# amirhajibabaei/AutoForce

Measured on AMD Instinct MI355X. Metric: MD-step atoms*steps/sec (SGPR predict: NL + descriptors + K_nm + E/F/stress + covloss); `value`: a Langevin MD loop on the device, every step from the forces of the one before (sgpr_md_run; --steps dependent steps between two fences); `value_resident_frames`: steps over independent frames resident i, higher is better.
Workload: dtype f64

## Files before the change

### autoforce_amd/csrc/api.hip

```cpp
#include <math.h>
#include <stdarg.h>
#include <stdio.h>
#include <stdlib.h>
#include <string.h>

#include <algorithm>
#include <numeric>

#include <dlfcn.h>
#include <unistd.h>
#include <rccl/rccl.h>

#include "../../include/sgpr_hip.h"
#include "sgpr_internal.h"
#include "nl_grid.inc"
#include <cmath>
#include <limits>

static thread_local char g_err[512] = "";
static int fail(int code, const char *fmt, ...)
{
    va_list ap;
    va_start(ap, fmt);
    vsnprintf(g_err, sizeof(g_err), fmt, ap);
// ... 1242 lines not shown
    if (const char *e = getenv("SGPR_ROWS16_MB")) h->rows16_mb = std::max(1, atoi(e));
    if (const char *e = getenv("SGPR_ROWS16_MIN")) h->rows16_min = std::max(1, atoi(e));
    {
        int ncu = 0;
        if (hipDeviceGetAttribute(&ncu, hipDeviceAttributeMultiprocessorCount, h->device) == hipSuccess && ncu >= 8) h->cus_per_xcd = ncu / 8;
    }
    if (getenv("SGPR_STAMPS")) { h->d_stamps.alloc(8 * 4096); h->d_stamps2.alloc(8 * 8192); }
    if (const char *e = getenv("SGPR_QR_KEEP")) h->qr_keep_mode = std::min(std::max(atoi(e), 0), 2);
    *out = h;
    return SGPR_OK;
}

static void drop_graph(sgpr_model *h)
{
    if (h->gexec) (void)hipGraphExecDestroy(h->gexec);
    h->gexec = nullptr;
}

extern "C" void sgpr_destroy(sgpr_model *h)
{
    if (!h) return;
    (void)hipSetDevice(h->device);
    (void)hipDeviceSynchronize();
    if (h->d_stamps.p && h->t_knm.n) {
        std::vector<long long> st(8 * h->t_knm.n);
        (void)hipMemcpy(st.data(), h->d_stamps.p, sizeof(long long) * st.size(), hipMemcpyDeviceToHost);
        double pro = 0, loop = 0, epi = 0; int n = 0; long long t0 = 1LL << 62, t1 = 0;
        for (size_t b = 0; b < h->t_knm.n; b++) {
            if (st[8 * b + 3] <= 0) continue;
            loop += st[8 * b + 1] - st[8 * b]; epi += st[8 * b + 2] - st[8 * b + 1]; n++;
            t0 = std::min(t0, st[8 * b]); t1 = std::max(t1, st[8 * b + 2]);
        }
        fprintf(stderr, "[sgpr stamps] K_nm gemm: %d tiles, start->loop end %.0f cyc, epilogue %.0f cyc, first start->last end %lld cyc\n",
                n, loop / std::max(n, 1), epi / std::max(n, 1), t1 - t0);
        (void)pro;
        if (const char *path = getenv("SGPR_STAMPS_FILE")) {
            if (FILE *f = fopen(path, "w")) {
                for (size_t b = 0; b < h->t_knm.n; b++)
                    fprintf(f, "knm %zu %lld %lld %lld %lld %lld %lld\n", b, st[8 * b], st[8 * b + 1], st[8 * b + 2], st[8 * b + 3], st[8 * b + 4], st[8 * b + 5]);
                std::vector<long long> s2(8 * std::min<size_t>(h->t_wcov.n, 8192));
                if (h->d_stamps2.p && !s2.empty()) {
                    (void)hipMemcpy(s2.data(), h->d_stamps2.p, sizeof(long long) * s2.size(), hipMemcpyDeviceToHost);
                    for (size_t b = 0; b < s2.size() / 8; b++)
                        fprintf(f, "wcov %zu %lld %lld %lld %lld %lld %lld\n", b, s2[8 * b], s2[8 * b + 1], s2[8 * b + 2], s2[8 * b + 3], s2[8 * b + 4], s2[8 * b + 5]);
                }
                fclose(f);
            }
        }
    }
    if (h->d_pstamps.p && h->N > 0) {
        const int N = h->N;
        std::vector<long long> st((size_t)16 * N);
        (void)hipMemcpy(st.data(), h->d_pstamps.p, sizeof(long long) * st.size(), hipMemcpyDeviceToHost);
        for (int pass = 0; pass < 2; pass++) {
            double d[7] = {0, 0, 0, 0, 0, 0, 0};
            long long t0 = 1LL << 62, t1 = 0;
            int cntw = 0;
            const int np = pass == 0 ? 6 : 3;
            for (int i = 0; i < h->cnt; i++) {
                const long long *w = st.data() + ((size_t)pass * N + i) * 8;
                if (w[0] <= 0 || w[np - 1] <= 0) continue;
                for (int k = 0; k + 1 < np; k++) d[k] += (double)(w[k + 1] - w[k]);
                t0 = std::min(t0, w[0]); t1 = std::max(t1, w[np - 1]);
                cntw++;
            }
            fprintf(stderr, "[sgpr stamps] %s: %d waves, cycles per phase:", pass == 0 ? "list+forward (sweep, sort, list out, tiles, c+spectrum)" : "reverse (dE/dc, pairs)", cntw);
            for (int k = 0; k + 1 < np; k++) fprintf(stderr, " %.0f", d[k] / std::max(cntw, 1));
            fprintf(stderr, "; first start -> last end %lld\n", t1 - t0);
            if (pass == 0) {
                double e[3] = {0, 0, 0};
                for (int i = 0; i < h->cnt; i++) {
                    const long long *w = st.data() + (size_t)i * 8;
                    if (w[0] <= 0 || w[5] <= 0) continue;
                    e[0] += (double)(w[3] - w[0]); e[1] += (double)(w[4] - w[3]); e[2] += (double)(w[5] - w[4]);
                }
                fprintf(stderr, "[sgpr stamps]    as a reuse step: list filter %.0f | c (radial, harmonics, MFMA) %.0f | spectrum + rows out %.0f\n",
                        e[0] / std::max(cntw, 1), e[1] / std::max(cntw, 1), e[2] / std::max(cntw, 1));
            }
        }
    }
    h->d_pstamps.release();
    drop_graph(h);
    for (auto e : h->ev) (void)hipEventDestroy(e);
    DevBuf<int> *ib[] = {&h->d_ind_slot, &h->d_ind_nn, &h->d_qoff, &h->d_perm, &h->d_slot, &h->d_aoff, &h->d_lslot,
                         &h->d_lnn, &h->d_bin_of, &h->d_bin_count, &h->d_nn_raw, &h->d_nn,
                         &h->d_nbr_j, &h->d_nbr_shift, &h->d_stat, &h->d_shear, &h->d_kslot, &h->d_aux,
                         &h->d_flag, &h->d_ncand, &h->d_cand_j, &h->d_cand_code, &h->d_cidx};
    for (auto b : ib) b->release();
    DevBuf<double> *db[] = {&h->d_radii, &h->d_Pm, &h->d_PmT, &h->d_pm_norm, &h->d_M, &h->d_mu, &h->d_choli,
                            &h->d_vs_sqrt, &h->d_gpart, &h->d_pos_in, &h->d_cell_in, &h->d_pos, &h->d_Pn, &h->d_norm, &h->d_C, &h->d_prec, &h->d_G,
                            &h->d_K, &h->d_Aw, &h->d_W, &h->d_F, &h->d_virpart, &h->d_Epart, &h->d_csq, &h->d_packed,
                            &h->d_rows_ones, &h->d_rows_out, &h->d_rows_ke, &h->d_L, &h->d_R1, &h->d_edit_tmp,
                            &h->d_rows_bG, &h->d_rows_bF, &h->d_rows_bV, &h->d_rows_kepart, &h->d_design, &h->d_qr_A, &h->d_qr_work};
    for (auto b : db) b->release();
    h->d_rows_cols.release();
    h->d_rows_rowof.release(); h->d_rows_qoff.release(); h->d_rows_vpart.release();
    if (h->pin) (void)hipHostFree(h->pin);
    if (h->pin_old) (void)hipHostFree(h->pin_old);
    if (h->md.halt_host) (void)hipHostFree(h->md.halt_host);
    if (h->md.mark) (void)hipHostFree(h->md.mark);
    if (h->md.scal_pin) (void)hipHostFree(h->md.scal_pin);
    {
        MdState &m = h->md;
        DevBuf<double> *mdb[] = {&m.X, &m.V, &m.P, &m.KE, &m.mass, &m.sig, &m.noise, &m.noise_raw, &m.cell, &m.scal_d};
        for (auto b : mdb) b->release();
        m.halt.release();
// ... 1615 lines not shown
```

### autoforce_amd/csrc/descriptor.hip

```cpp
#include "sgpr_internal.h"
#include "gemm_tile.inc"

__constant__ HarmCoef c_hc;

void upload_harm_coef(const HarmCoef &hc) { (void)hipMemcpyToSymbol(HIP_SYMBOL(c_hc), &hc, sizeof(HarmCoef)); }

#define SQRT2 1.4142135623730951
typedef double v4d __attribute__((ext_vector_type(4)));

__device__ __forceinline__ void wave_sync()
{
    __builtin_amdgcn_fence(__ATOMIC_RELEASE, "wavefront");
    __builtin_amdgcn_wave_barrier();
    __builtin_amdgcn_fence(__ATOMIC_ACQUIRE, "wavefront");
}

__device__ __forceinline__ double uniform(double v)
{
    const int lo = __builtin_amdgcn_readfirstlane(__double2loint(v));
    const int hi = __builtin_amdgcn_readfirstlane(__double2hiint(v));
    return __hiloint2double(hi, lo);
}

template <typename T>
__device__ __forceinline__ const T *launder(const T *p)
{
    asm volatile("" : "+s"(p));
    return p;
}

__device__ __forceinline__ double wave_sum(double v)
{
#pragma unroll
    for (int o = 32; o > 0; o >>= 1) v += __shfl_xor(v, o, 64);
    return v;
}

__device__ __forceinline__ int xcd_quad(int b, int n, int R)
{
    if (R <= 0) return b;
    const int grp = 8 * R, g0 = b / grp * grp;
    if (g0 + grp > n) return b;
    const int r = b - g0;
    return g0 + (r & 7) * R + (r >> 3);
}

template <int LMAX>
struct Harm {
    static constexpr int L1 = LMAX + 1, LL = L1 * L1;
    double A[L1], B[L1], q[L1][L1];
    double x, y, z, rho;
    const HarmCoef *hc = &c_hc;

    __device__ __forceinline__ void prepare(double x_, double y_, double z_)
    {
        x = x_; y = y_; z = z_;
        rho = x * x + y * y + z * z;
        A[0] = 1.0; B[0] = 0.0;
#pragma unroll
        for (int m = 1; m <= LMAX; m++) {
            A[m] = x * A[m - 1] - y * B[m - 1];
            B[m] = y * A[m - 1] + x * B[m - 1];
        }
        q[0][0] = hc->y00;
#pragma unroll
        for (int l = 1; l <= LMAX; l++) {
#pragma unroll
            for (int m = 0; m <= l - 2; m++)
                q[l][m] = hc->al[l][m] * (z * q[l - 1][m] + rho * hc->bl[l][m] * q[l - 2][m]);
            q[l][l - 1] = hc->cl[l] * z * q[l - 1][l - 1];
            q[l][l] = hc->dl[l] * q[l - 1][l - 1];
        }
    }

    __device__ __forceinline__ void eval(double x_, double y_, double z_, double *Y)
    {
        prepare(x_, y_, z_);
#pragma unroll
        for (int l = 0; l <= LMAX; l++) {
            Y[l * l] = q[l][0];
#pragma unroll
// ... 174 lines not shown

template <bool ENV>
__device__ __forceinline__ void load_neighbor(const DescArgs &a, int gi, int ia, int t, const double *pi,
                                              const double *cell, double r[3], int &s, int &j)
{
    if constexpr (ENV) {
        const int64_t e = a.env_ptr[ia] + t;
        r[0] = a.env_r[3 * e]; r[1] = a.env_r[3 * e + 1]; r[2] = a.env_r[3 * e + 2];
        s = a.env_slot[e];
        j = -1;
    } else {
        const size_t e = (size_t)gi * a.maxnn + t;
        j = a.nbr_j[e];
        const int code = a.nbr_shift[e];
        const double s0 = (double)(int)(int8_t)(code & 0xff);
        const double s1 = (double)(int)(int8_t)((code >> 8) & 0xff);
        const double s2 = (double)(int)(int8_t)((code >> 16) & 0xff);
#pragma unroll
        for (int k = 0; k < 3; k++)
            r[k] = a.pos[3 * (size_t)j + k] - pi[k] + (s0 * cell[k] + s1 * cell[3 + k] + s2 * cell[6 + k]);
        s = (code >> 24) & 0xff;
    }
}

template <int NMAX>
__device__ __forceinline__ void radial_ex(double d, double u, double rc, double irc, double ex, double *f, double &g,
                                          double &dg)
{
    const double ud = u * d;
    const double step = ud < rc ? 1.0 : 0.0;
    const double qq = 1.0 - ud * irc;
    const double cut = step * qq * qq;
    const double dcut = step * (-2.0 * qq * irc) * u;
    g = cut * ex;
    dg = dcut * ex - d * g;
    const double rho = d * d;
    double pw = g;
#pragma unroll
    for (int n = 0; n <= NMAX; n++) { f[n] = pw; pw *= rho; }
}

template <int NMAX>
__device__ __forceinline__ void radial(double d, double u, double rc, double *f, double &g, double &dg, double &ex)
{
    ex = exp(-0.5 * d * d);
    radial_ex<NMAX>(d, u, rc, 1.0 / rc, ex, f, g, dg);
}

template <int LMAX, int NMAX>
struct WaveLds {
    static constexpr int L1 = LMAX + 1, N1 = NMAX + 1, LL = L1 * L1, LLP = LL + 1, NSLOT = N1 * LL;
    static constexpr int CH = 48;
    static constexpr int TILE_D = CH * N1 + CH * LLP;
};

template <int LMAX, int NMAX, int ST, bool ENV>
__global__ __launch_bounds__(256) void desc_fwd_kernel(DescArgs a)
{
    using WL = WaveLds<LMAX, NMAX>;
    constexpr int N1 = WL::N1, LL = WL::LL, LLP = WL::LLP, NSLOT = WL::NSLOT;
    constexpr int SPL = (NSLOT + 63) / 64;
    extern __shared__ double smem[];
    const int wave = threadIdx.x >> 6, lane = threadIdx.x & 63;
    const int ia = blockIdx.x * 4 + wave;
    if (ia >= a.N) return;
    const int gi = a.first + ia * a.stride;
    constexpr int CH = WL::CH;
    const int perwave = WL::TILE_D + ST * NSLOT + 64 / 2;
    double *fl = smem + (size_t)wave * perwave;
    double *Yl = fl + CH * N1;
    double *cl = Yl + CH * LLP;
    int *sl = (int *)(cl + ST * NSLOT);

    int nn;
    double pi[3] = {0, 0, 0}, cell[9];
    if constexpr (ENV) {
        nn = (int)(a.env_ptr[ia + 1] - a.env_ptr[ia]);
    } else {
        nn = a.nn[gi];
#pragma unroll
        for (int k = 0; k < 3; k++) pi[k] = a.pos[3 * (size_t)gi + k];
#pragma unroll
        for (int k = 0; k < 9; k++) cell[k] = a.cell[k];
    }

    bool shear = false;
    if (nn > CH) {
        bool near = false;
        for (int t0 = 0; t0 < nn; t0 += 64) {
            const int t = t0 + lane;
            if (t < nn) {
                double r[3]; int s, j;
                load_neighbor<ENV>(a, gi, ia, t, pi, cell, r, s, j);
                const double u = unit_of<ST>(a, s);
                const double tol = SGPR_TINY_ANGLE * fabs(r[2] / u);
                near |= (fabs(r[0] / u) < tol) && (fabs(r[1] / u) < tol);
            }
        }
        shear = __any(near);
    }

    double acc[ST][SPL];
#pragma unroll
    for (int s = 0; s < ST; s++)
#pragma unroll
        for (int k = 0; k < SPL; k++) acc[s][k] = 0.0;
// ... 106 lines not shown
                nrm2 += pv[k][l] * pv[k][l];
            }
        }
    }
    nrm2 = wave_sum(nrm2);
    const double nrm = sqrt(nrm2);
    const double inv = nn > 0 ? 1.0 / (nrm + SGPR_EPS) : 0.0;
#pragma unroll
    for (int k = 0; k < MAXP; k++) {
        const int pr = lane + 64 * k;
        if (pr < npair) {
#pragma unroll
            for (int l = 0; l < L1; l++) a.Pn[(size_t)ia * a.Dpad + pr * L1 + l] = pv[k][l] * inv;
        }
    }
    for (int e = a.Dc + lane; e < a.Dpad; e += 64) a.Pn[(size_t)ia * a.Dpad + e] = 0.0;
    if (lane == 0) {
        a.norm[ia] = nn > 0 ? nrm : 0.0;
        if (a.shear) a.shear[ia] = shear ? 1 : 0;
    }
}

#define NL_SORT_MAX 256
#ifndef NL_STEPS
#define NL_STEPS 4
#endif

struct NlArgs {
    const NlGrid *grid;
    const int *bin_of, *kslot, *bin_count;
    int cap;
    const BinRec *b_rec;
    const BinAux *b_aux;
    int *nn, *nn_local, *nn_raw, *nbr_j, *nbr_shift, *aux;
    unsigned short *T;
    int t_stride;
    int *stat;
    const int *flag;
    double rc_list;
    int *ncand, *cand_j, *cand_code, *cidx;
    unsigned long long *hm;
    int hmw;
};

#ifdef SGPR_PHASE_STAMPS
#define PHASE_STAMP(K) if (a.stamps && lane == 0) a.stamps[(size_t)ia * 8 + (K)] = (long long)__builtin_amdgcn_s_memtime()
#else
#define PHASE_STAMP(K)
#endif

template <int LMAX, int NMAX, int ST>
struct FwdLds {
    using WL = WaveLds<LMAX, NMAX>;
    static constexpr int CH = WL::CH;
    static constexpr int BINL = NL_SORT_MAX + NL_SORT_MAX / 2, HIT0 = BINL + 2 * 64;
    static constexpr int NLV = HIT0 + 4 * CH;
    static constexpr int FWV = CH * WL::N1 + CH * WL::LLP + CH / 2;
    static constexpr int P4V = ST * WL::NSLOT;
    static constexpr int RA = (NLV > FWV ? (NLV > P4V ? NLV : P4V) : (FWV > P4V ? FWV : P4V));
    static constexpr int PW = 4 * CH + RA;
};

template <int LMAX, int NMAX, int ST>
__global__ __launch_bounds__(256, 4) void nl_fwd_kernel(DescArgs a, NlArgs n)
{
    using WL = WaveLds<LMAX, NMAX>;
    using FL = FwdLds<LMAX, NMAX, ST>;
    constexpr int N1 = WL::N1, LL = WL::LL, LLP = WL::LLP, NSLOT = WL::NSLOT, CH = WL::CH;
    constexpr int UC = ST * N1, CBS = (UC + 15) / 16, RBL = (LL + 15) / 16;
    extern __shared__ double smem[];
    const int wave = __builtin_amdgcn_readfirstlane(threadIdx.x >> 6), lane = threadIdx.x & 63;
    const int ia = xcd_quad((int)blockIdx.x, (int)gridDim.x, a.xq) * 4 + wave;
    if (ia >= a.N) return;
    const int i = a.first + ia * a.stride;
    double *wbase = smem + (size_t)wave * FL::PW;
    double *hit1 = wbase;
    double *RA = wbase + 4 * CH;
    unsigned long long *keys = (unsigned long long *)RA;
    int *hq = (int *)(RA + NL_SORT_MAX);
    int4 *binl = (int4 *)(RA + FL::BINL);
    double *hit0 = RA + FL::HIT0;
    double *fl = RA;
    double *Yl = fl + CH * N1;
    int *sl = (int *)(Yl + CH * LLP);
    double *cl = RA;

    PHASE_STAMP(0);
    const int cap = n.cap, maxnn = a.maxnn;
    double h[9];
#pragma unroll
    for (int k = 0; k < 9; k++) h[k] = a.cell[k];
    const double xi = uniform(a.pos[3 * (size_t)i]), yi = uniform(a.pos[3 * (size_t)i + 1]), zi = uniform(a.pos[3 * (size_t)i + 2]);
    const int ki = __builtin_amdgcn_readfirstlane(n.kslot[i]);
    const bool ghost = ki < 0;
    const unsigned long long lt = lane == 0 ? 0ull : (~0ull >> (64 - lane));
    const bool rebuild = __builtin_amdgcn_readfirstlane(*n.flag) != 0;
    int ncand = 0;
    int j_first = 0, cd_first = 0;
    if (rebuild) {
        const NlGrid g = *n.grid;
        const int bi = __builtin_amdgcn_readfirstlane(n.bin_of[i]);
        int wi0 = 0, wi1 = 0, wi2 = 0;
        if (ki >= 0 && ki < cap) {
            const BinAux own = n.b_aux[(size_t)bi * cap + ki];
            wi0 = own.w0; wi1 = own.w1; wi2 = own.w2;
        }
        auto fdiv = [](int q, float inv) { return (int)(((float)q + 0.5f) * inv); };
        const float i_n2 = 1.0f / (float)g.nb[2], i_n1 = 1.0f / (float)g.nb[1];
        const int bq = fdiv(bi, i_n2);
        const int b2 = bi - bq * g.nb[2];
        const int b0 = fdiv(bq, i_n1);
        const int b1 = bq - b0 * g.nb[1];
        const int w0 = 2 * g.rng[0] + 1, w1 = 2 * g.rng[1] + 1, w2 = 2 * g.rng[2] + 1;
        const float i_w2 = 1.0f / (float)w2, i_w1 = 1.0f / (float)w1;
        const double r_n0 = 1.0 / g.nb[0], r_n1 = 1.0 / g.nb[1], r_n2 = 1.0 / g.nb[2];
        const int nbox = w0 * w1 * w2;
        const bool t_ok = n.T != nullptr && (long long)nbox * cap <= (long long)n.t_stride && cap <= 4096 && maxnn <= 65535 &&
                          ki < cap && !ghost;
        if (n.T != nullptr && !t_ok && ki < cap && !ghost && lane == 0)
            atomicMax(&n.stat[2], cap <= 4096 && maxnn <= 65535 ? nbox * cap : 0x7fffffff);
        const int grp = lane >> 4, s16 = lane & 15;
        const double rl2 = n.rc_list * n.rc_list;
        int base = 0;
        auto consume = [&](bool valid, const BinRec &rec, const BinAux &ax, int code, int q, int k) {
            bool hit = false;
            int f0 = 0, f1 = 0, f2 = 0;
            if (valid) {
                f0 = (int)(int8_t)(code & 0xff) - ax.w0 + wi0;
                f1 = (int)(int8_t)((code >> 8) & 0xff) - ax.w1 + wi1;
                f2 = (int)(int8_t)((code >> 16) & 0xff) - ax.w2 + wi2;
                const double dx = rec.x - xi + (f0 * h[0] + f1 * h[3] + f2 * h[6]);
                const double dy = rec.y - yi + (f0 * h[1] + f1 * h[4] + f2 * h[7]);
                const double dz = rec.z - zi + (f0 * h[2] + f1 * h[5] + f2 * h[8]);
                hit = dx * dx + dy * dy + dz * dz < rl2 && !(rec.idx == i && f0 == 0 && f1 == 0 && f2 == 0);
            }
            const unsigned long long m = __ballot(hit);
            if (hit) {
// ... 140 lines not shown
            n.ncand[i] = ncand;
            n.nn_raw[ia] = base;
        }
        if (ncand > NL_SORT_MAX) __threadfence();
        PHASE_STAMP(2);
    } else {
        const int nc_v = n.ncand[i];
        if (lane < maxnn) {
            const size_t e = (size_t)i * maxnn + lane;
            j_first = n.cand_j[e];
            cd_first = n.cand_code[e];
        }
        ncand = __builtin_amdgcn_readfirstlane(nc_v);
        if (lane == 0) n.nn_raw[ia] = ncand;
    }
    const double rc2_lo = a.rc * a.rc * (1.0 - 1e-14), rc2_hi = a.rc * a.rc * (1.0 + 1e-14);
    int nn = 0;
    bool near = false;
    for (int c0 = 0; c0 < ncand; c0 += 64) {
        const int c = c0 + lane;
        bool hit = false;
        int j = 0, cd = 0;
        double r0 = 1.0, r1 = 0.0, r2 = 0.0;
        if (c < ncand) {
            if (rebuild && c < NL_SORT_MAX) {
                const unsigned long long key = keys[c];
                const unsigned img = (unsigned)(key >> 16) & 0xffffffu;
                const int f0 = (int)((img >> 16) & 0xff) - 128, f1 = (int)((img >> 8) & 0xff) - 128, f2 = (int)(img & 0xff) - 128;
                j = (int)(key >> 40);
                cd = (f0 & 0xff) | ((f1 & 0xff) << 8) | ((f2 & 0xff) << 16) | (((int)(key >> 12) & 0xf) << 24);
            } else if (!rebuild && c0 == 0) {
                j = j_first; cd = cd_first;
            } else {
                const size_t e = (size_t)i * maxnn + c;
                j = n.cand_j[e];
                cd = n.cand_code[e];
            }
            const int f0 = (int)(int8_t)(cd & 0xff), f1 = (int)(int8_t)((cd >> 8) & 0xff), f2 = (int)(int8_t)((cd >> 16) & 0xff);
            r0 = a.pos[3 * (size_t)j] - xi + (f0 * h[0] + f1 * h[3] + f2 * h[6]);
            r1 = a.pos[3 * (size_t)j + 1] - yi + (f0 * h[1] + f1 * h[4] + f2 * h[7]);
            r2 = a.pos[3 * (size_t)j + 2] - zi + (f0 * h[2] + f1 * h[5] + f2 * h[8]);
            const double d2 = r0 * r0 + r1 * r1 + r2 * r2;
            hit = d2 < rc2_lo || (d2 < rc2_hi && sqrt(d2) < a.rc);
        }
        const unsigned long long m = __ballot(hit);
        if (lane == 0) n.hm[(size_t)i * n.hmw + (c0 >> 6)] = m;
        if (hit) {
            const int t = nn + __popcll(m & lt);
            const int sj = (cd >> 24) & 0xff;
            const size_t e = (size_t)i * maxnn + t;
            n.nbr_j[e] = j;
            n.nbr_shift[e] = cd;
            n.cidx[e] = c;
            double *dst = t < CH ? hit0 + 4 * t : (t < 2 * CH ? hit1 + 4 * (t - CH) : nullptr);
            if (dst) { dst[0] = r0; dst[1] = r1; dst[2] = r2; dst[3] = __hiloint2double(0, sj); }
            const double tol = SGPR_TINY_ANGLE * fabs(r2);
            near |= (fabs(r0) < tol) && (fabs(r1) < tol);
        }
        nn += __popcll(m);
    }
    for (int w = (ncand + 63) / 64 + lane; w < n.hmw; w += 64) n.hm[(size_t)i * n.hmw + w] = 0ull;
    const bool shear = __any(near);
    if (lane == 0) {
        n.nn[i] = nn;
        n.nn_local[ia] = nn;
    }
    wave_sync();
    double h0r[3] = {1.0, 0.0, 0.0};
    int h0s = 0;
    if (lane < min(nn, CH)) {
        h0r[0] = hit0[4 * lane]; h0r[1] = hit0[4 * lane + 1]; h0r[2] = hit0[4 * lane + 2];
        h0s = __double2loint(hit0[4 * lane + 3]);
    }
    if (nn > 2 * CH) __threadfence();
    PHASE_STAMP(3);
    v4d D[RBL][CBS];
#pragma unroll
    for (int rb = 0; rb < RBL; rb++)
#pragma unroll
        for (int cb = 0; cb < CBS; cb++) D[rb][cb] = (v4d){0.0, 0.0, 0.0, 0.0};
    const double ang = shear ? SGPR_TINY_ANGLE : 0.0;
    for (int t0 = 0; t0 < nn; t0 += CH) {
        const int cnt = min(CH, nn - t0);
        const bool on = lane < cnt;
        const int t = t0 + lane;
        double r[3] = {1.0, 0.0, 0.0};
        int s = 0;
        if (on) {
            if (t0 == 0) { r[0] = h0r[0]; r[1] = h0r[1]; r[2] = h0r[2]; s = h0s; }
            else if (t0 == CH) {
                r[0] = hit1[4 * lane]; r[1] = hit1[4 * lane + 1]; r[2] = hit1[4 * lane + 2];
                s = __double2loint(hit1[4 * lane + 3]);
            } else {
                const size_t e = (size_t)i * maxnn + t;
                const int j = n.nbr_j[e];
                const int cd = n.nbr_shift[e];
                const int f0 = (int)(int8_t)(cd & 0xff), f1 = (int)(int8_t)((cd >> 8) & 0xff), f2 = (int)(int8_t)((cd >> 16) & 0xff);
                s = (cd >> 24) & 0xff;
                r[0] = a.pos[3 * (size_t)j] - xi + (f0 * h[0] + f1 * h[3] + f2 * h[6]);
                r[1] = a.pos[3 * (size_t)j + 1] - yi + (f0 * h[1] + f1 * h[4] + f2 * h[7]);
                r[2] = a.pos[3 * (size_t)j + 2] - zi + (f0 * h[2] + f1 * h[5] + f2 * h[8]);
            }
        }
        const double u = unit_of<ST>(a, s);
        const double iu = inv_unit_of<ST>(a, s);
        const double x = r[0] * iu, y = r[1] * iu, z = r[2] * iu;
        const double d = sqrt(x * x + y * y + z * z);
        double f[N1], gg, dg;
        const double ex = exp(-0.5 * d * d);
        radial_ex<NMAX>(d, u, a.rc, a.irc, ex, f, gg, dg);
        double Y[LL];
        Harm<LMAX> hm;
        hm.eval(x, y - ang * z, ang * y + z, Y);
        if (on && a.prec) {
            double2 *dst = (double2 *)(a.prec + ((size_t)i * maxnn + t) * 4);
            dst[0] = make_double2(r[0], r[1]);
            dst[1] = make_double2(r[2], ex);
        }
        wave_sync();
        if (lane < CH) {
#pragma unroll
            for (int q = 0; q < N1; q++) fl[lane * N1 + q] = on ? f[q] : 0.0;
#pragma unroll
            for (int k = 0; k < LL; k++) Yl[lane * LLP + k] = on ? Y[k] : 0.0;
            sl[lane] = on ? s : -1;
        }
        wave_sync();
        for (int g16 = 0; g16 < cnt; g16 += 16) {
            double av[4][RBL], bv[4][CBS];
#pragma unroll
            for (int q = 0; q < 4; q++) {
                const int tr = g16 + 4 * q + (lane >> 4);
                const int st = sl[tr];
#pragma unroll
                for (int rb = 0; rb < RBL; rb++) {
                    const int lm = 16 * rb + (lane & 15);
                    av[q][rb] = (RBL * 16 == LL || lm < LL) ? Yl[tr * LLP + (lm < LL ? lm : 0)] : 0.0;
                }
#pragma unroll
                for (int cb = 0; cb < CBS; cb++) {
                    const int c = 16 * cb + (lane & 15);
                    const double fv = fl[tr * N1 + (c < UC ? c % N1 : 0)];
                    bv[q][cb] = (c < UC && st == c / N1) ? fv : 0.0;
                }
            }
#pragma unroll
            for (int q = 0; q < 4; q++)
#pragma unroll
                for (int rb = 0; rb < RBL; rb++)
#pragma unroll
                    for (int cb = 0; cb < CBS; cb++)
                        D[rb][cb] = __builtin_amdgcn_mfma_f64_16x16x4f64(av[q][rb], bv[q][cb], D[rb][cb], 0, 0, 0);
        }
    }
    wave_sync();
    PHASE_STAMP(4);
    constexpr int L1 = LMAX + 1;
    constexpr int UMAX = ST * N1;
    constexpr bool PMF = UMAX <= 16;
    constexpr int CLS = PMF ? LL + 1 : LL;
#pragma unroll
    for (int rb = 0; rb < RBL; rb++)
#pragma unroll
        for (int cb = 0; cb < CBS; cb++)
#pragma unroll
            for (int q = 0; q < 4; q++) {
                const int lm = 16 * rb + (lane >> 4) + 4 * q, c = 16 * cb + (lane & 15);
                if ((RBL * 16 == LL || lm < LL) && (CBS * 16 == UC || c < UC)) {
                    const int idx = (c / N1) * NSLOT + (c % N1) * LL + lm;
                    cl[PMF ? c * CLS + lm : idx] = D[rb][cb][q];
                }
            }
    wave_sync();
    if (a.C)
        for (int idx = lane; idx < species_in_use<LMAX, NMAX, ST>(a) * NSLOT; idx += 64)
            a.C[(size_t)ia * a.CS + idx] = cl[PMF ? (idx / LL) * CLS + idx % LL : idx];
    double nrm2 = 0.0;
    const int npair = a.Dc / L1;
    if constexpr (PMF) {
        const int Ur = species_in_use<LMAX, NMAX, ST>(a) * N1, vch = lane & 15;
        double cf[L1][4];
        int eidx[4];
#pragma unroll
        for (int r = 0; r < 4; r++) {
            const int u = (lane >> 4) + 4 * r;
            const bool keep = u <= vch && vch < Ur;
            eidx[r] = keep ? (u * Ur - (u * (u - 1)) / 2 + (vch - u)) * L1 : -1;
#pragma unroll
            for (int l = 0; l < L1; l++) cf[l][r] = keep ? a.pack[eidx[r] + l].coef : 0.0;
        }
// ... 28 lines not shown
        for (int e = a.Dc + lane; e < a.Dpad; e += 64) a.Pn[(size_t)ia * a.Dpad + e] = 0.0;
        if (lane == 0) {
            a.norm[ia] = nn > 0 ? nrm : 0.0;
            if (a.shear) a.shear[ia] = shear ? 1 : 0;
        }
        PHASE_STAMP(5);
        return;
    }
    constexpr int MAXP = ((UMAX * (UMAX + 1)) / 2 + 63) / 64;
    double pv[MAXP][L1];
#pragma unroll
    for (int k = 0; k < MAXP; k++) {
        const int pr = lane + 64 * k;
#pragma unroll
        for (int l = 0; l < L1; l++) pv[k][l] = 0.0;
        if (pr < npair) {
            const PackEntry p0 = a.pack[pr * L1];
            const double *cu = cl + (p0.u / N1) * NSLOT + (p0.u % N1) * LL;
            const double *cv = cl + (p0.v / N1) * NSLOT + (p0.v % N1) * LL;
#pragma unroll
            for (int l = 0; l < L1; l++) {
                double sacc = 0.0;
#pragma unroll
                for (int mm = 0; mm < 2 * l + 1; mm++) sacc += cu[l * l + mm] * cv[l * l + mm];
                pv[k][l] = sacc * a.pack[pr * L1 + l].coef;
                nrm2 += pv[k][l] * pv[k][l];
            }
        }
    }
    nrm2 = wave_sum(nrm2);
    const double nrm = sqrt(nrm2);
    const double inv = nn > 0 ? 1.0 / (nrm + SGPR_EPS) : 0.0;
#pragma unroll
    for (int k = 0; k < MAXP; k++) {
        const int pr = lane + 64 * k;
        if (pr < npair) {
#pragma unroll
            for (int l = 0; l < L1; l++) a.Pn[(size_t)ia * a.Dpad + pr * L1 + l] = pv[k][l] * inv;
        }
    }
    for (int e = a.Dc + lane; e < a.Dpad; e += 64) a.Pn[(size_t)ia * a.Dpad + e] = 0.0;
    if (lane == 0) {
        a.norm[ia] = nn > 0 ? nrm : 0.0;
        if (a.shear) a.shear[ia] = shear ? 1 : 0;
    }
    PHASE_STAMP(5);
}

template <int LMAX, int NMAX>
struct RevDims {
    static constexpr int N1 = NMAX + 1, L1 = LMAX + 1, LL = L1 * L1, NSLOT = N1 * LL;
    static constexpr int KS = (N1 + 3) / 4;
    static constexpr int CB = (LL + 15) / 16;
    static constexpr int CH = 48, RB = CH / 16;
    static constexpr int SP = LL | 1;
    static constexpr int FS = 8 * KS + 1;
};

template <int LMAX, int NMAX, int ST>
static int rev_region_doubles(int Dpad)
{
    using RD = RevDims<LMAX, NMAX>;
    const int UT = ST * RD::N1;
    const int dc = ST * RD::NSLOT + (ST <= 4 ? UT * UT * RD::L1 : Dpad);
    int r = RD::CH * RD::SP;
    if (RD::CH * RD::FS > r) r = RD::CH * RD::FS;
    if (12 * RD::CH > r) r = 12 * RD::CH;
    if (dc > r) r = dc;
    return (r + 1) & ~1;
}

template <int LMAX, int NMAX, int ST, bool GATHER, bool ROWS, bool COV = false>
__global__ __launch_bounds__(256, 4) void desc_rev_kernel(DescArgs a, GemmArgs gc, int n_cov)
{
    extern __shared__ double smem[];
    const int S_use = species_in_use<LMAX, NMAX, ST>(a);
    if constexpr (COV) {
        if ((int)blockIdx.x < n_cov) {
            using GL = GemmLds<EPI_ROWSQ, 1, 16>;
            gemm_tile_body<EPI_ROWSQ, 1, 16>(gc, (int)blockIdx.x, smem, smem + GL::NBUF * GL::ASZ);
            return;
        }
    }
    const int bx = COV ? (int)blockIdx.x - n_cov : (int)blockIdx.x;
    const int nbx = COV ? (int)gridDim.x - n_cov : (int)gridDim.x;
    const double *const rows_aw = ROWS ? a.rows_aw : nullptr;
    using RD = RevDims<LMAX, NMAX>;
    constexpr int N1 = RD::N1, L1 = RD::L1, LL = RD::LL, NSLOT = RD::NSLOT;
    constexpr int KS = RD::KS, CB = RD::CB, CH = RD::CH, RB = RD::RB, SP = RD::SP, FS = RD::FS;
    constexpr int SPL = (NSLOT + 63) / 64;
    constexpr int WPW = SGPR_REV_WPW(ST);
    __shared__ double vred[4][9];
    const int wave = __builtin_amdgcn_readfirstlane(threadIdx.x >> 6), lane = threadIdx.x & 63;
    const int qd = xcd_quad(bx, nbx, a.xq);
    const int ia = qd * WPW + wave;
    const bool active = ia < a.N;
    const int perwave = ST * NSLOT + a.rsz + CH / 2;
    double *dcl = smem + (size_t)wave * perwave;
    double *R = dcl + ST * NSLOT;
    int *sl = (int *)(R + a.rsz);
    const int gi = a.first + (active ? ia : 0) * a.stride;
    const int bq = ROWS ? a.rows_cols[blockIdx.y] : 0;
    const bool off_species = ROWS && active && a.slot[gi] != a.rows_colslot[bq];
    const int nn = (active && !off_species) ? a.nn[gi] : 0;
    const double aw_q = (ROWS && active) ? rows_aw[(size_t)ia * a.rows_ld + bq] : 1.0;
    double *Gb = a.G, *Fnbr_b = a.Fnbr, *Fself_b = a.Fself, *vir_b = a.vir_part;
    if constexpr (ROWS) {
        if (Gb) Gb += blockIdx.y * a.g_stride;
        if (Fnbr_b) Fnbr_b += blockIdx.y * a.f_stride;
        if (Fself_b) Fself_b += blockIdx.y * a.f_stride;
        vir_b += blockIdx.y * a.v_stride;
    }
    double tot = 0.0;
    bool zero_dc = false;

    PHASE_STAMP(0);
    constexpr int MAXE_H = ((ST * RD::N1 * (ST * RD::N1 + 1)) / 2 * RD::L1 + 63) / 64;
    constexpr bool HOIST = MAXE_H <= 10;
    const double nrm_h = active ? a.norm[ia] : 0.0;
    double wv_h[HOIST ? MAXE_H : 1], pv_h[HOIST ? MAXE_H : 1], cv_h[HOIST ? ST * SPL : 1];
    PackEntry pe_h[HOIST ? MAXE_H : 1];
    if constexpr (HOIST) {
        const double *Wi = ROWS ? a.rows_pm + (size_t)bq * a.Dpad : a.W + (size_t)(active ? ia : 0) * a.Dpad;
        const double *Pi = a.Pn + (size_t)(active ? ia : 0) * a.Dpad;
#pragma unroll
        for (int k = 0; k < MAXE_H; k++) {
            const int e = lane + 64 * k;
            const bool in = e < a.Dc && active;
            wv_h[k] = in ? aw_q * Wi[e] : 0.0;
            pv_h[k] = in ? Pi[e] : 0.0;
            pe_h[k] = a.pack[in ? e : 0];
        }
#pragma unroll
        for (int s = 0; s < ST; s++)
#pragma unroll
            for (int k = 0; k < SPL; k++) {
                const int slot = lane + 64 * k;
                cv_h[s * SPL + k] = (active && s < S_use && (SPL * 64 == NSLOT || slot < NSLOT)) ? a.C[(size_t)ia * a.CS + s * NSLOT + slot] : 0.0;
            }
    }
    if (nn > 0) {
        const double nrm = nrm_h;
        if (!(nrm > 0.0) || (ROWS && aw_q == 0.0)) {
            for (int k = lane; k < ST * NSLOT; k += 64) dcl[k] = 0.0;
            zero_dc = true;
        } else {
            const int Ur = S_use * N1;
            constexpr bool EXPAND = ST <= 4;
            constexpr int UT = ST * N1;
            double *cl = R;
            double *gl = R + ST * NSLOT;
            const double sden = nrm + SGPR_EPS;
            constexpr int MAXE = ((UT * (UT + 1)) / 2 * L1 + 63) / 64;
// ... 94 lines not shown
                        dcl[s * NSLOT + slot] = d;
                    }
                }
            }
        }
        PHASE_STAMP(1);
        const double ang = a.shear[ia] ? SGPR_TINY_ANGLE : 0.0;
        double *stage = R;
        int nn_b = nn;
        if constexpr (ROWS) {
            if (a.slot[gi] != a.rows_colslot[bq]) nn_b = 0;
        }
        for (int t0 = 0; t0 < nn_b; t0 += CH) {
            const int cnt = min(CH, nn_b - t0);
            const bool on = lane < cnt;
            const int t = t0 + lane;
            double r[3] = {1.0, 0.0, 0.0}, ex = 0.0;
            int s = 0, j = 0, rvp = 0;
            if (on) {
                const size_t e = (size_t)gi * a.maxnn + t;
                const double2 *src = (const double2 *)(a.prec + e * 4);
                const double2 p0 = src[0], p1 = src[1];
                r[0] = p0.x; r[1] = p0.y; r[2] = p1.x; ex = p1.y;
                s = (a.nbr_shift[e] >> 24) & 0xff;
                j = a.nbr_j[e];
                if constexpr (GATHER) {
                    const int c = min(max(a.cidx[e], 0), a.maxnn - 1);
                    const int hs = min(max(a.aux[(size_t)gi * a.maxnn + c], 0), a.t_stride - 1);
                    const int cr = min((int)a.T[(size_t)gi * a.t_stride + hs], a.maxnn - 1);
                    const unsigned long long *hj = a.hm + (size_t)j * a.hmw;
                    int pcount = __popcll(hj[cr >> 6] & ((1ull << (cr & 63)) - 1ull));
                    for (int w = 0; w < (cr >> 6); w++) pcount += __popcll(hj[w]);
                    rvp = min(pcount, a.maxnn - 1);
                }
            }
            if (zero_dc) {
                if constexpr (GATHER) {
                    if (on) {
                        double2 *dst = (double2 *)(Gb + ((size_t)j * a.maxnn + rvp) * 4);
                        dst[0] = make_double2(0.0, 0.0);
                        dst[1] = make_double2(0.0, 0.0);
                    }
                }
                continue;
            }
            const double u = unit_of<ST>(a, s);
            const double iu = inv_unit_of<ST>(a, s);
            const double x = r[0] * iu, y = r[1] * iu, z = r[2] * iu;
            const double d = sqrt(x * x + y * y + z * z);
            const double id = 1.0 / d;
            double f[N1], g, dg;
            radial_ex<NMAX>(d, u, a.rc, a.irc, ex, f, g, dg);
            wave_sync();
            if (on) {
                double rpow = 1.0;
                const double rho = d * d;
#pragma unroll
                for (int n = 0; n < 4 * KS; n++) {
                    stage[lane * FS + n] = n < N1 ? f[n < N1 ? n : 0] : 0.0;
                    stage[lane * FS + 4 * KS + n] = n < N1 ? dg * rpow + (n ? g * 2.0 * n * rpow * id : 0.0) : 0.0;
                    rpow *= rho;
                }
            }
            if (lane < CH) sl[lane] = on ? s : -1;
            wave_sync();
            double af[RB][KS], ah[RB][KS];
            int sr[RB];
#pragma unroll
            for (int rb = 0; rb < RB; rb++) {
                const int row = 16 * rb + (lane & 15);
                sr[rb] = sl[row];
#pragma unroll
                for (int ks = 0; ks < KS; ks++) {
                    af[rb][ks] = stage[row * FS + 4 * ks + (lane >> 4)];
                    ah[rb][ks] = stage[row * FS + 4 * KS + 4 * ks + (lane >> 4)];
                }
            }
            wave_sync();
            Harm<LMAX> h;
            h.hc = launder(&c_hc);
            h.prepare(x, y - ang * z, ang * y + z);
            double dEdd = 0.0, gxs = 0.0, gys = 0.0, gzs = 0.0;
#pragma unroll
            for (int pass = 0; pass < 2; pass++) {
#pragma unroll
                for (int cb = 0; cb < CB; cb++) {
                    const int n_b = lane >> 4, lm = 16 * cb + (lane & 15);
#pragma unroll
                    for (int rb = 0; rb < RB; rb++) {
                        v4d D = (v4d){0.0, 0.0, 0.0, 0.0};
                        for (int sp = 0; sp < S_use; sp++) {
                            if (__ballot(sr[rb] == sp) == 0ull) continue;
#pragma unroll
                            for (int ks = 0; ks < KS; ks++) {
                                const int n = 4 * ks + n_b;
                                const bool ok = n < N1 && lm < LL;
                                const double bv = dcl[sp * NSLOT + (ok ? n * LL + lm : 0)];
                                const double av = pass == 0 ? ah[rb][ks] : af[rb][ks];
                                D = __builtin_amdgcn_mfma_f64_16x16x4f64(sr[rb] == sp ? av : 0.0, ok ? bv : 0.0, D, 0, 0, 0);
                            }
                        }
                        if (CB * 16 == LL || lm < LL) {
#pragma unroll
                            for (int q = 0; q < 4; q++) stage[(16 * rb + (lane >> 4) + 4 * q) * SP + lm] = D[q];
                        }
                    }
                }
                wave_sync();
                if (on) {
                    if (pass == 0) dEdd = h.dot(stage + lane * SP);
                    else {
                        h.hc = launder(h.hc);
                        h.backward(stage + lane * SP, gxs, gys, gzs);
                    }
                }
                wave_sync();
            }
            const double rad = dEdd * id;
            double gr[3];
            gr[0] = (gxs + rad * x) * iu;
            gr[1] = (gys + ang * gzs + rad * y) * iu;
            gr[2] = (-ang * gys + gzs + rad * z) * iu;
            if (on) {
                if constexpr (GATHER) {
                    double2 *dst = (double2 *)(Gb + ((size_t)j * a.maxnn + rvp) * 4);
                    dst[0] = make_double2(gr[0], gr[1]);
                    dst[1] = make_double2(gr[2], 0.0);
                } else {
#pragma unroll
                    for (int k = 0; k < 3; k++) {
                        if (!(fabs(gr[k]) < SGPR_FIX_LIMIT) && a.stat) atomicMax(&a.stat[3], 3);
                        atomicAdd((unsigned long long *)&Fnbr_b[3 * (size_t)j + k], (unsigned long long)__double2ll_rn(-gr[k] * SGPR_FIX_SCALE));
                    }
                }
            }
            if (lane < CH) {
                const double rv[3] = {x * u, y * u, z * u};
#pragma unroll
                for (int p = 0; p < 3; p++)
#pragma unroll
                    for (int q = 0; q < 3; q++) stage[(3 * p + q) * CH + lane] = on ? rv[p] * gr[q] : 0.0;
#pragma unroll
                for (int k = 0; k < 3; k++) stage[(9 + k) * CH + lane] = on ? gr[k] : 0.0;
            }
            wave_sync();
            if (lane < 48) {
                const double *src = stage + (lane >> 2) * CH + (lane & 3) * (CH / 4);
                double sacc = 0.0;
#pragma unroll
                for (int i = 0; i < CH / 4; i++) sacc += src[i];
                tot += sacc;
            }
        }
    }
    PHASE_STAMP(2);
    tot += __shfl_xor(tot, 1, 64);
    tot += __shfl_xor(tot, 2, 64);
    if (lane < 48 && (lane & 3) == 0) {
        const int k = lane >> 2;
        if (k < 9) vred[wave][k] = tot;
        else if (active) Fself_b[3 * (size_t)gi + (k - 9)] = tot;
    }
    __syncthreads();
    if (wave == 0 && lane < 9)
        vir_b[(size_t)lane * nbx + qd] = WPW == 1 ? vred[0][lane] : vred[0][lane] + vred[1][lane] + vred[2][lane] + vred[3][lane];
}

__global__ void unpack_kernel(int n, int S, int L1, int N1, int Dc, int Dpad, const PackEntry *pack,
                              const double *Pp, double *Pd)
{
    const int i = blockIdx.x;
    const int D = N1 * N1 * L1;
    for (int e = threadIdx.x; e < Dc; e += blockDim.x) {
        const PackEntry pe = pack[e];
        const int su = pe.u / N1, nu = pe.u % N1, sv = pe.v / N1, nv = pe.v % N1;
        const double v = Pp[(size_t)i * Dpad + e] / (pe.u == pe.v ? 1.0 : SQRT2);
        double *base = Pd + (size_t)i * S * S * D;
        base[((size_t)sv * S + su) * D + (nu * N1 + nv) * L1 + pe.l] = v;
        base[((size_t)su * S + sv) * D + (nv * N1 + nu) * L1 + pe.l] = v;
    }
}

void launch_unpack_descriptors(int n, int S, int lmax, int nmax, int Dc, int Dpad, const PackEntry *pack,
                               const double *Pp, double *Pdense, hipStream_t st)
{
    if (n <= 0) return;
    hipLaunchKernelGGL(unpack_kernel, dim3(n), dim3(128), 0, st, n, S, lmax + 1, nmax + 1, Dc, Dpad, pack, Pp, Pdense);
}

template <int LMAX, int NMAX, int ST>
static size_t fwd_lds_bytes()
{
    using WL = WaveLds<LMAX, NMAX>;
    return sizeof(double) * 4 * (size_t)(WL::TILE_D + ST * WL::NSLOT + 32);
}

template <int LMAX, int NMAX, int ST, bool ENV>
static int run_fwd(const DescArgs &a, hipStream_t st)
{
    if (a.N <= 0) return 0;
    const size_t lds = fwd_lds_bytes<LMAX, NMAX, ST>();
    static bool attr_set = false;
    if (!attr_set) {
        (void)hipFuncSetAttribute((const void *)desc_fwd_kernel<LMAX, NMAX, ST, ENV>,
                                  hipFuncAttributeMaxDynamicSharedMemorySize, (int)lds);
        attr_set = true;
    }
    hipLaunchKernelGGL((desc_fwd_kernel<LMAX, NMAX, ST, ENV>), dim3((a.N + 3) / 4), dim3(256), lds, st, a);
    return 0;
}

template <int LMAX, int NMAX, int ST>
static int run_bwd(DescArgs a, hipStream_t st, const GemmParams *cov = nullptr)
{
    if (a.N <= 0) return 0;
    using RD = RevDims<LMAX, NMAX>;
    a.rsz = rev_region_doubles<LMAX, NMAX, ST>(a.Dpad);
    constexpr int WPW = SGPR_REV_WPW(ST);
    if (WPW == 1) a.xq = 0;
    size_t lds = sizeof(double) * WPW * (size_t)(ST * RD::NSLOT + a.rsz + RD::CH / 2);
    static size_t attr_set[6] = {0, 0, 0, 0, 0, 0};
    const bool gather = a.G != nullptr, rows = a.rows_aw != nullptr;
    const bool with_cov = WPW == 4 && cov && !rows && cov->tiles && cov->ntiles > 0 && cov->bm == 32 && cov->kd == 16;
    GemmArgs gc = {};
    int n_cov = 0;
    if (with_cov) {
        gc.p = *cov;
        gc.ieta = -1;
        n_cov = cov->ntiles;
        lds = std::max(lds, sizeof(double) * (size_t)GemmLds<EPI_ROWSQ, 1, 16>::DOUBLES);
    }
    const int which = with_cov ? 4 + gather : 2 * gather + rows;
    const void *fn = with_cov ? (gather ? (const void *)desc_rev_kernel<LMAX, NMAX, ST, true, false, true>
                                        : (const void *)desc_rev_kernel<LMAX, NMAX, ST, false, false, true>)
                   : gather ? (rows ? (const void *)desc_rev_kernel<LMAX, NMAX, ST, true, true>
                                    : (const void *)desc_rev_kernel<LMAX, NMAX, ST, true, false>)
                            : (rows ? (const void *)desc_rev_kernel<LMAX, NMAX, ST, false, true>
                                    : (const void *)desc_rev_kernel<LMAX, NMAX, ST, false, false>);
    if (attr_set[which] < lds) {
        (void)hipFuncSetAttribute(fn, hipFuncAttributeMaxDynamicSharedMemorySize, (int)lds);
        attr_set[which] = lds;
    }
    const dim3 grid((a.N + WPW - 1) / WPW + n_cov, rows ? a.batch : 1), blk(64 * WPW);
    if (with_cov && gather) hipLaunchKernelGGL((desc_rev_kernel<LMAX, NMAX, ST, true, false, true>), grid, blk, lds, st, a, gc, n_cov);
    else if (with_cov) hipLaunchKernelGGL((desc_rev_kernel<LMAX, NMAX, ST, false, false, true>), grid, blk, lds, st, a, gc, n_cov);
    else if (gather && rows) hipLaunchKernelGGL((desc_rev_kernel<LMAX, NMAX, ST, true, true>), grid, blk, lds, st, a, gc, n_cov);
    else if (gather) hipLaunchKernelGGL((desc_rev_kernel<LMAX, NMAX, ST, true, false>), grid, blk, lds, st, a, gc, n_cov);
    else if (rows) hipLaunchKernelGGL((desc_rev_kernel<LMAX, NMAX, ST, false, true>), grid, blk, lds, st, a, gc, n_cov);
    else hipLaunchKernelGGL((desc_rev_kernel<LMAX, NMAX, ST, false, false>), grid, blk, lds, st, a, gc, n_cov);
    return 0;
}

static int st_of(int S) { return S <= 1 ? 1 : S <= 2 ? 2 : S <= 3 ? 3 : S <= 4 ? 4 : S <= 8 ? 8 : 16; }

#define DISPATCH_LNS(FN, ...)                                                              \
    do {                                                                                   \
        const int stv = st_of(p.S);                                                        \
        if (p.lmax == 3 && p.nmax == 3) {                                                  \
            if (stv == 1) return FN(3, 3, 1, __VA_ARGS__);                                  \
            if (stv == 2) return FN(3, 3, 2, __VA_ARGS__);                                  \
            if (stv == 3) return FN(3, 3, 3, __VA_ARGS__);                                  \
            if (stv == 4) return FN(3, 3, 4, __VA_ARGS__);                                  \
            if (stv == 8) return FN(3, 3, 8, __VA_ARGS__);                                  \
            return FN(3, 3, 16, __VA_ARGS__);                                               \
        }                                                                                  \
        if (stv > 8) return -6;                                                                                     \
        if (p.lmax == 2 && p.nmax == 2) {                                                  \
            if (stv <= 2) return FN(2, 2, 2, __VA_ARGS__);                                  \
            if (stv <= 4) return FN(2, 2, 4, __VA_ARGS__);                                  \
            return FN(2, 2, 8, __VA_ARGS__);                                                \
        }                                                                                  \
        if (p.lmax == 4 && p.nmax == 4) {                                                  \
            if (stv <= 2) return FN(4, 4, 2, __VA_ARGS__);                                  \
// ... 105 lines not shown
```

Before: 49.15 million.

## Widen neighbor chunk to full wave and swizzle LDS staging in forward/reverse kernels

Raises the per-iteration neighbor chunk from 48 to 64 so every lane of the wave does useful work in both the forward list+descriptor kernel and the reverse kernel. It also XOR-swizzles and skews the LDS harmonic staging rows to avoid bank conflicts, and replaces species LDS slots with shuffles or packed bytes. The second hit buffer is dropped to keep LDS usage in check. The cost is fewer hits kept in LDS (more global reloads when a neighbor list exceeds one chunk) and extra index arithmetic. A stamps dump to file is also added for profiling.

```diff
diff --git a/autoforce_amd/csrc/api.hip b/autoforce_amd/csrc/api.hip
--- a/autoforce_amd/csrc/api.hip
+++ b/autoforce_amd/csrc/api.hip
@@ -1318,6 +1318,19 @@
         const int N = h->N;
         std::vector<long long> st((size_t)16 * N);
         (void)hipMemcpy(st.data(), h->d_pstamps.p, sizeof(long long) * st.size(), hipMemcpyDeviceToHost);
+        if (const char *path = getenv("SGPR_PSTAMPS_FILE")) {
+            std::vector<int> nnh(h->d_nn.n, 0);
+            if (!nnh.empty()) (void)hipMemcpy(nnh.data(), h->d_nn.p, sizeof(int) * nnh.size(), hipMemcpyDeviceToHost);
+            if (FILE *f = fopen(path, "w")) {
+                for (int i = 0; i < h->cnt; i++) {
+                    const size_t gi = (size_t)h->rank + (size_t)i * h->world;
+                    const long long *fw = st.data() + (size_t)i * 8, *rv = st.data() + ((size_t)N + i) * 8;
+                    fprintf(f, "%d %d %lld %lld %lld %lld %lld %lld %lld %lld %lld\n", i, gi < nnh.size() ? nnh[gi] : -1, fw[0], fw[1], fw[2],
+                            fw[3], fw[4], fw[5], rv[0], rv[1], rv[2]);
+                }
+                fclose(f);
+            }
+        }
         for (int pass = 0; pass < 2; pass++) {
             double d[7] = {0, 0, 0, 0, 0, 0, 0};
             long long t0 = 1LL << 62, t1 = 0;
diff --git a/autoforce_amd/csrc/descriptor.hip b/autoforce_amd/csrc/descriptor.hip
--- a/autoforce_amd/csrc/descriptor.hip
+++ b/autoforce_amd/csrc/descriptor.hip
@@ -27,6 +27,12 @@
 {
     asm volatile("" : "+s"(p));
     return p;
+}
+
+__device__ __forceinline__ int opaque(int v)
+{
+    asm volatile("" : "+v"(v));
+    return v;
 }
 
 __device__ __forceinline__ double wave_sum(double v)
@@ -307,6 +313,11 @@
     static constexpr int L1 = LMAX + 1, N1 = NMAX + 1, LL = L1 * L1, LLP = LL + 1, NSLOT = N1 * LL;
     static constexpr int CH = 48;
     static constexpr int TILE_D = CH * N1 + CH * LLP;
+    static constexpr int CHS = 64;
+    static constexpr bool SWZ = LL == 16;
+    static constexpr int RS = SWZ ? LL : (LL | 1);
+    static __device__ __forceinline__ int rot(int row) { return (row ^ (row >> 4)) & 15; }
+    static __device__ __forceinline__ int at(int row, int k) { return SWZ ? row * RS + (k ^ rot(row)) : row * RS + k; }
 };
 
 template <int LMAX, int NMAX, int ST, bool ENV>
@@ -519,13 +530,13 @@
 template <int LMAX, int NMAX, int ST>
 struct FwdLds {
     using WL = WaveLds<LMAX, NMAX>;
-    static constexpr int CH = WL::CH;
+    static constexpr int CH = WL::CHS;
     static constexpr int BINL = NL_SORT_MAX + NL_SORT_MAX / 2, HIT0 = BINL + 2 * 64;
     static constexpr int NLV = HIT0 + 4 * CH;
-    static constexpr int FWV = CH * WL::N1 + CH * WL::LLP + CH / 2;
-    static constexpr int P4V = ST * WL::NSLOT;
+    static constexpr int FWV = CH * WL::N1 + CH * WL::RS;
+    static constexpr int P4V = ST * WL::NSLOT + 16;
     static constexpr int RA = (NLV > FWV ? (NLV > P4V ? NLV : P4V) : (FWV > P4V ? FWV : P4V));
-    static constexpr int PW = 4 * CH + RA;
+    static constexpr int PW = RA;
 };
 
 template <int LMAX, int NMAX, int ST>
@@ -533,7 +544,7 @@
 {
     using WL = WaveLds<LMAX, NMAX>;
     using FL = FwdLds<LMAX, NMAX, ST>;
-    constexpr int N1 = WL::N1, LL = WL::LL, LLP = WL::LLP, NSLOT = WL::NSLOT, CH = WL::CH;
+    constexpr int N1 = WL::N1, LL = WL::LL, NSLOT = WL::NSLOT, CH = WL::CHS;
     constexpr int UC = ST * N1, CBS = (UC + 15) / 16, RBL = (LL + 15) / 16;
     extern __shared__ double smem[];
     const int wave = __builtin_amdgcn_readfirstlane(threadIdx.x >> 6), lane = threadIdx.x & 63;
@@ -541,15 +552,13 @@
     if (ia >= a.N) return;
     const int i = a.first + ia * a.stride;
     double *wbase = smem + (size_t)wave * FL::PW;
-    double *hit1 = wbase;
-    double *RA = wbase + 4 * CH;
+    double *RA = wbase;
     unsigned long long *keys = (unsigned long long *)RA;
     int *hq = (int *)(RA + NL_SORT_MAX);
     int4 *binl = (int4 *)(RA + FL::BINL);
     double *hit0 = RA + FL::HIT0;
     double *fl = RA;
     double *Yl = fl + CH * N1;
-    int *sl = (int *)(Yl + CH * LLP);
     double *cl = RA;
 
     PHASE_STAMP(0);
@@ -796,7 +805,7 @@
             n.nbr_j[e] = j;
             n.nbr_shift[e] = cd;
             n.cidx[e] = c;
-            double *dst = t < CH ? hit0 + 4 * t : (t < 2 * CH ? hit1 + 4 * (t - CH) : nullptr);
+            double *dst = t < CH ? hit0 + 4 * t : nullptr;
             if (dst) { dst[0] = r0; dst[1] = r1; dst[2] = r2; dst[3] = __hiloint2double(0, sj); }
             const double tol = SGPR_TINY_ANGLE * fabs(r2);
             near |= (fabs(r0) < tol) && (fabs(r1) < tol);
@@ -816,7 +825,7 @@
         h0r[0] = hit0[4 * lane]; h0r[1] = hit0[4 * lane + 1]; h0r[2] = hit0[4 * lane + 2];
         h0s = __double2loint(hit0[4 * lane + 3]);
     }
-    if (nn > 2 * CH) __threadfence();
+    if (nn > CH) __threadfence();
     PHASE_STAMP(3);
     v4d D[RBL][CBS];
 #pragma unroll
@@ -832,10 +841,7 @@
         int s = 0;
         if (on) {
             if (t0 == 0) { r[0] = h0r[0]; r[1] = h0r[1]; r[2] = h0r[2]; s = h0s; }
-            else if (t0 == CH) {
-                r[0] = hit1[4 * lane]; r[1] = hit1[4 * lane + 1]; r[2] = hit1[4 * lane + 2];
-                s = __double2loint(hit1[4 * lane + 3]);
-            } else {
+            else {
                 const size_t e = (size_t)i * maxnn + t;
                 const int j = n.nbr_j[e];
                 const int cd = n.nbr_shift[e];
@@ -862,24 +868,22 @@
             dst[1] = make_double2(r[2], ex);
         }
         wave_sync();
-        if (lane < CH) {
-#pragma unroll
-            for (int q = 0; q < N1; q++) fl[lane * N1 + q] = on ? f[q] : 0.0;
-#pragma unroll
-            for (int k = 0; k < LL; k++) Yl[lane * LLP + k] = on ? Y[k] : 0.0;
-            sl[lane] = on ? s : -1;
-        }
+#pragma unroll
+        for (int q = 0; q < N1; q++) fl[lane * N1 + q] = on ? f[q] : 0.0;
+#pragma unroll
+        for (int k = 0; k < LL; k++) Yl[WL::at(lane, k)] = on ? Y[k] : 0.0;
+        const int sv = on ? s : -1;
         wave_sync();
         for (int g16 = 0; g16 < cnt; g16 += 16) {
             double av[4][RBL], bv[4][CBS];
 #pragma unroll
             for (int q = 0; q < 4; q++) {
                 const int tr = g16 + 4 * q + (lane >> 4);
-                const int st = sl[tr];
+                const int st = __shfl(sv, tr, 64);
 #pragma unroll
                 for (int rb = 0; rb < RBL; rb++) {
                     const int lm = 16 * rb + (lane & 15);
-                    av[q][rb] = (RBL * 16 == LL || lm < LL) ? Yl[tr * LLP + (lm < LL ? lm : 0)] : 0.0;
+                    av[q][rb] = (RBL * 16 == LL || lm < LL) ? Yl[WL::at(tr, lm < LL ? lm : 0)] : 0.0;
                 }
 #pragma unroll
                 for (int cb = 0; cb < CBS; cb++) {
@@ -1014,8 +1018,11 @@
     static constexpr int N1 = NMAX + 1, L1 = LMAX + 1, LL = L1 * L1, NSLOT = N1 * LL;
     static constexpr int KS = (N1 + 3) / 4;
     static constexpr int CB = (LL + 15) / 16;
-    static constexpr int CH = 48, RB = CH / 16;
+    static constexpr int CH = WaveLds<LMAX, NMAX>::CHS, RB = CH / 16;
+    static constexpr bool SKEW = LL == 16;
     static constexpr int SP = LL | 1;
+    static constexpr int STAGE = SKEW ? CH * LL + CH / 2 : CH * SP;
+    static __device__ __forceinline__ int at(int row) { return SKEW ? row * LL + (row >> 1) : row * SP; }
     static constexpr int FS = 8 * KS + 1;
 };
 
@@ -1025,7 +1032,7 @@
     using RD = RevDims<LMAX, NMAX>;
     const int UT = ST * RD::N1;
     const int dc = ST * RD::NSLOT + (ST <= 4 ? UT * UT * RD::L1 : Dpad);
-    int r = RD::CH * RD::SP;
+    int r = RD::STAGE;
     if (RD::CH * RD::FS > r) r = RD::CH * RD::FS;
     if (12 * RD::CH > r) r = 12 * RD::CH;
     if (dc > r) r = dc;
@@ -1057,10 +1064,10 @@
     const int qd = xcd_quad(bx, nbx, a.xq);
     const int ia = qd * WPW + wave;
     const bool active = ia < a.N;
-    const int perwave = ST * NSLOT + a.rsz + CH / 2;
+    const int perwave = ST * NSLOT + a.rsz + CH / 8;
     double *dcl = smem + (size_t)wave * perwave;
     double *R = dcl + ST * NSLOT;
-    int *sl = (int *)(R + a.rsz);
+    unsigned char *sl = (unsigned char *)(R + a.rsz);
     const int gi = a.first + (active ? ia : 0) * a.stride;
     const int bq = ROWS ? a.rows_cols[blockIdx.y] : 0;
     const bool off_species = ROWS && active && a.slot[gi] != a.rows_colslot[bq];
@@ -1261,75 +1268,82 @@
             double f[N1], g, dg;
             radial_ex<NMAX>(d, u, a.rc, a.irc, ex, f, g, dg);
             wave_sync();
+            const int ln = opaque(lane);
             if (on) {
                 double rpow = 1.0;
                 const double rho = d * d;
 #pragma unroll
                 for (int n = 0; n < 4 * KS; n++) {
-                    stage[lane * FS + n] = n < N1 ? f[n < N1 ? n : 0] : 0.0;
-                    stage[lane * FS + 4 * KS + n] = n < N1 ? dg * rpow + (n ? g * 2.0 * n * rpow * id : 0.0) : 0.0;
+                    stage[ln * FS + n] = n < N1 ? f[n < N1 ? n : 0] : 0.0;
+                    stage[ln * FS + 4 * KS + n] = n < N1 ? dg * rpow + (n ? g * 2.0 * n * rpow * id : 0.0) : 0.0;
                     rpow *= rho;
                 }
             }
-            if (lane < CH) sl[lane] = on ? s : -1;
+            sl[(ln & 15) * RB + (ln >> 4)] = (unsigned char)(on ? s : 0xff);
             wave_sync();
             double af[RB][KS], ah[RB][KS];
-            int sr[RB];
+            static_assert(RB == 4, "species bytes of a lane's rows fill one word");
+            const int la = opaque(lane);
+            const unsigned srp = ((const unsigned *)sl)[la & 15];
 #pragma unroll
             for (int rb = 0; rb < RB; rb++) {
-                const int row = 16 * rb + (lane & 15);
-                sr[rb] = sl[row];
+                const int row = 16 * rb + (la & 15);
 #pragma unroll
                 for (int ks = 0; ks < KS; ks++) {
-                    af[rb][ks] = stage[row * FS + 4 * ks + (lane >> 4)];
-                    ah[rb][ks] = stage[row * FS + 4 * KS + 4 * ks + (lane >> 4)];
+                    af[rb][ks] = stage[row * FS + 4 * ks + (la >> 4)];
+                    ah[rb][ks] = stage[row * FS + 4 * KS + 4 * ks + (la >> 4)];
                 }
             }
             wave_sync();
             Harm<LMAX> h;
             h.hc = launder(&c_hc);
             h.prepare(x, y - ang * z, ang * y + z);
-            double dEdd = 0.0, gxs = 0.0, gys = 0.0, gzs = 0.0;
+            double rad = 0.0, gxs = 0.0, gys = 0.0, gzs = 0.0;
 #pragma unroll
             for (int pass = 0; pass < 2; pass++) {
 #pragma unroll
                 for (int cb = 0; cb < CB; cb++) {
-                    const int n_b = lane >> 4, lm = 16 * cb + (lane & 15);
+                    const int lp = opaque(lane);
+                    const int n_b = lp >> 4, lm = 16 * cb + (lp & 15);
 #pragma unroll
                     for (int rb = 0; rb < RB; rb++) {
                         v4d D = (v4d){0.0, 0.0, 0.0, 0.0};
+                        const int sr_rb = (int)((srp >> (8 * rb)) & 0xffu);
                         for (int sp = 0; sp < S_use; sp++) {
-                            if (__ballot(sr[rb] == sp) == 0ull) continue;
+                            if (__ballot(sr_rb == sp) == 0ull) continue;
 #pragma unroll
                             for (int ks = 0; ks < KS; ks++) {
                                 const int n = 4 * ks + n_b;
                                 const bool ok = n < N1 && lm < LL;
                                 const double bv = dcl[sp * NSLOT + (ok ? n * LL + lm : 0)];
                                 const double av = pass == 0 ? ah[rb][ks] : af[rb][ks];
-                                D = __builtin_amdgcn_mfma_f64_16x16x4f64(sr[rb] == sp ? av : 0.0, ok ? bv : 0.0, D, 0, 0, 0);
+                                D = __builtin_amdgcn_mfma_f64_16x16x4f64(sr_rb == sp ? av : 0.0, ok ? bv : 0.0, D, 0, 0, 0);
                             }
                         }
                         if (CB * 16 == LL || lm < LL) {
 #pragma unroll
-                            for (int q = 0; q < 4; q++) stage[(16 * rb + (lane >> 4) + 4 * q) * SP + lm] = D[q];
+                            for (int q = 0; q < 4; q++) stage[RD::at(lp >> 4) + lm + RD::at(16 * rb + 4 * q)] = D[q];
                         }
                     }
                 }
                 wave_sync();
                 if (on) {
-                    if (pass == 0) dEdd = h.dot(stage + lane * SP);
+                    const double *row = stage + RD::at(opaque(lane));
+                    if (pass == 0) rad = h.dot(row) * id;
                     else {
                         h.hc = launder(h.hc);
-                        h.backward(stage + lane * SP, gxs, gys, gzs);
+                        h.backward(row, gxs, gys, gzs);
                     }
                 }
                 wave_sync();
             }
-            const double rad = dEdd * id;
+            int s_again = s;
+            asm volatile("" : "+v"(s_again));
+            const double u_e = unit_of<ST>(a, s_again), iu_e = inv_unit_of<ST>(a, s_again);
             double gr[3];
-            gr[0] = (gxs + rad * x) * iu;
-            gr[1] = (gys + ang * gzs + rad * y) * iu;
-            gr[2] = (-ang * gys + gzs + rad * z) * iu;
+            gr[0] = (gxs + rad * x) * iu_e;
+            gr[1] = (gys + ang * gzs + rad * y) * iu_e;
+            gr[2] = (-ang * gys + gzs + rad * z) * iu_e;
             if (on) {
                 if constexpr (GATHER) {
                     double2 *dst = (double2 *)(Gb + ((size_t)j * a.maxnn + rvp) * 4);
@@ -1343,22 +1357,30 @@
                     }
                 }
             }
-            if (lane < CH) {
-                const double rv[3] = {x * u, y * u, z * u};
+            const int lv = opaque(lane);
+            {
+                const double rv[3] = {x * u_e, y * u_e, z * u_e};
 #pragma unroll
                 for (int p = 0; p < 3; p++)
 #pragma unroll
-                    for (int q = 0; q < 3; q++) stage[(3 * p + q) * CH + lane] = on ? rv[p] * gr[q] : 0.0;
-#pragma unroll
-                for (int k = 0; k < 3; k++) stage[(9 + k) * CH + lane] = on ? gr[k] : 0.0;
+                    for (int q = 0; q < 3; q++) stage[(3 * p + q) * CH + lv] = on ? rv[p] * gr[q] : 0.0;
+#pragma unroll
+                for (int k = 0; k < 3; k++) stage[(9 + k) * CH + lv] = on ? gr[k] : 0.0;
             }
             wave_sync();
             if (lane < 48) {
-                const double *src = stage + (lane >> 2) * CH + (lane & 3) * (CH / 4);
+                const double *src = stage + (lv >> 2) * CH + (lv & 3) * 12;
                 double sacc = 0.0;
 #pragma unroll
-                for (int i = 0; i < CH / 4; i++) sacc += src[i];
+                for (int i = 0; i < 12; i++) sacc += src[i];
                 tot += sacc;
+                if (cnt > 48) {
+                    const int r0 = 48 + (lv & 3) * 12;
+                    double sacc2 = 0.0;
+#pragma unroll
+                    for (int i = 0; i < 12; i++) sacc2 += r0 + i < CH ? src[48 + i] : 0.0;
+                    tot += sacc2;
+                }
             }
         }
     }
@@ -1427,7 +1449,7 @@
     a.rsz = rev_region_doubles<LMAX, NMAX, ST>(a.Dpad);
     constexpr int WPW = SGPR_REV_WPW(ST);
     if (WPW == 1) a.xq = 0;
-    size_t lds = sizeof(double) * WPW * (size_t)(ST * RD::NSLOT + a.rsz + RD::CH / 2);
+    size_t lds = sizeof(double) * WPW * (size_t)(ST * RD::NSLOT + a.rsz + RD::CH / 8);
     static size_t attr_set[6] = {0, 0, 0, 0, 0, 0};
     const bool gather = a.G != nullptr, rows = a.rows_aw != nullptr;
     const bool with_cov = WPW == 4 && cov && !rows && cov->tiles && cov->ntiles > 0 && cov->bm == 32 && cov->kd == 16;
```

Result: faster. 51.06 million, median of 6 (+3.9%).
